# ricosjp/FrontISTR

Hardware: AMD Instinct MI355X
Metric: CG iterations/sec + SpMV achieved HBM GB/s, 10M-DOF 3x3-block mesh (higher is better)
Workload: dtype f64

## Files before the change

### frontistr_amd/csrc/fistr_hip.hip

```cpp
#include <dlfcn.h>
#include <rccl/rccl.h>
#include <stdio.h>
#include <stdlib.h>
#include <string.h>

#include <algorithm>
#include <chrono>
#include <mutex>
#include <thread>

#include "fx_assemble.h"
#include "fx_assemble_tet.h"
#include "fx_assemble_c3.h"
#include "fx_kernels.h"
#include "fx_nonlinear.h"
#include "fx_nonlinear_tet.h"
#include "fx_nonlinear_c3.h"

namespace fxo {
struct Graph {
  int32_t n = 0;
  std::vector<int64_t> ptr;
  std::vector<int32_t> adj;
};
// ... 245 lines not shown
    {"FX_DF_GRID", [](fx_context *c, double v) { c->df_grid = (int)v; }},
    {"FX_DF_POLL", [](fx_context *c, double v) { c->df_poll = (int)v; }},
    {"FX_DF_SLEEP", [](fx_context *c, double v) { c->df_sleep = std::max(0, (int)v); }},
    {"FX_DF_PRESLEEP", [](fx_context *c, double v) { c->df_presleep = std::max(0, (int)v); }},
    {"FX_DF_WPS", [](fx_context *c, double v) { c->df_wps = ((int)v == 2 || (int)v == 4) ? (int)v : 8; }},
    {"FX_MARCH", [](fx_context *c, double v) { c->march_mode = std::max(0, std::min(2, (int)v)); }},
    {"FX_MARCH_CHUNK", [](fx_context *c, double v) { c->march_chunk = std::max(0, (int)v); }},
    {"FX_MARCH_WAVES", [](fx_context *c, double v) { c->march_waves = (int)v; }},
    {"FX_MARCH_GRID", [](fx_context *c, double v) { c->march_grid = std::max(0, (int)v); }},
    {"FX_MARCH_XCD", [](fx_context *c, double v) { c->march_xcd = (int)v != 0; }},
    {"FX_DEBUG_DF_FAIL", [](fx_context *c, double v) { c->dbg_df_fail = (int)v != 0; }},
    {"FX_DEBUG_ONECOLOR", [](fx_context *c, double v) { c->dbg_onecolor = (int)v != 0; }},
    {"FX_SSOR_NATURAL", [](fx_context *c, double v) { c->ssor_natural = (int)v != 0; }},
    {"FX_SPLIT_WPS", [](fx_context *c, double v) { c->split_wps = ((int)v == 2 || (int)v == 4 || (int)v == 8) ? (int)v : 0; }},
};

extern "C" int fx_set_option(fx_context *c, const char *name, double value) {
  if (!c || !name) { g_fx_error = "fx_set_option: null argument"; return FX_ERROR_RUNTIME; }
  for (const FxOption &o : g_fx_options)
    if (strcmp(o.name, name) == 0) {
      const bool spatial = c->spmv_spatial;
      const int bs = c->spmv_bs;
      o.set(c, value);
      if (c->m_symbolic && (spatial != c->spmv_spatial || bs != c->spmv_bs)) {
        HIP_TRY(hipSetDevice(c->device));
        HIP_TRY(hipStreamSynchronize(c->stream));
        return spmv_walk(c);
      }
      return 0;
    }
  g_fx_error = std::string("fx_set_option: unknown option ") + name;
  return FX_ERROR_UNSUPPORTED;
}
// ... 7 lines not shown
    const char *lr = getenv("LOCAL_RANK");
    if (!lr) lr = getenv("OMPI_COMM_WORLD_LOCAL_RANK");
    if (!lr) lr = getenv("MPI_LOCALRANKID");
    if (!lr) lr = getenv("SLURM_LOCALID");
    device = lr ? atoi(lr) % ndev : 0;
  }
  HIP_TRY(hipSetDevice(device));
  fx_context *c = new fx_context();
  c->device = device;
  HIP_TRY(hipDeviceGetAttribute(&c->n_cu, hipDeviceAttributeMultiprocessorCount, device));
  if (context_init(c)) {
    fx_destroy(c);
    return FX_ERROR_RUNTIME;
  }
  for (const FxOption &o : g_fx_options)
    if (const char *e = getenv(o.name)) o.set(c, atof(e));
  {
    int pc[3] = {64, 64, 64};
    auto occ = [&](int k, auto kernel, int threads) {
      int n = 0;
      if (hipOccupancyMaxActiveBlocksPerMultiprocessor(&n, kernel, threads, 0) != hipSuccess) n = 1;
      pc[k] = std::min(pc[k], n);
    };
    occ(0, k_tri_dataflow<2, 1, true>, 128); occ(0, k_tri_dataflow<2, 0, true>, 128); occ(0, k_tri_dataflow<2, 1, false>, 128); occ(0, k_tri_dataflow<2, 0, false>, 128);
    occ(1, k_tri_dataflow<4, 1, true>, 256); occ(1, k_tri_dataflow<4, 0, true>, 256); occ(1, k_tri_dataflow<4, 1, false>, 256); occ(1, k_tri_dataflow<4, 0, false>, 256);
    occ(2, k_tri_dataflow<8, 1, true>, 512); occ(2, k_tri_dataflow<8, 0, true>, 512); occ(2, k_tri_dataflow<8, 1, false>, 512); occ(2, k_tri_dataflow<8, 0, false>, 512);
    (void)hipGetLastError();
    for (int k = 0; k < 3; k++) c->df_grid_max[k] = std::max(1, c->n_cu * std::max(1, std::min(pc[k], 8)));
    int pe[2] = {1, 1};
    if (hipOccupancyMaxActiveBlocksPerMultiprocessor(&pe[0], k_eis_backward_df<4>, 256, 0) != hipSuccess) pe[0] = 1;
    if (hipOccupancyMaxActiveBlocksPerMultiprocessor(&pe[1], k_eis_forward_df<4>, 256, 0) != hipSuccess) pe[1] = 1;
    (void)hipGetLastError();
    for (int k = 0; k < 2; k++) c->eis_df_grid_max[k] = std::max(1, c->n_cu * std::max(1, std::min(pe[k], EIS_DF_MAX_PER_CU)));
    int pm[4] = {1, 1, 1, 1};
    auto occm = [&](int k, auto kernel, int threads) {
      if (hipOccupancyMaxActiveBlocksPerMultiprocessor(&pm[k], kernel, threads, 0) != hipSuccess) pm[k] = 1;
    };
    occm(0, k_tri_march<1>, 64 * 2); occm(1, k_tri_march<2>, 64 * 3); occm(2, k_tri_march<3>, 64 * 4); pm[3] = pm[2];
    (void)hipGetLastError();
    for (int k = 0; k < 4; k++) c->march_grid_max[k] = std::max(8, c->n_cu * std::max(1, std::min(pm[k], 4)));
  }
  *out = c;
  return 0;
}

static void arena_destroy(fx_context *c) {
// ... 1578 lines not shown
    const int s0 = S.color_slice[col], s1 = S.color_slice[col + 1];
    if (s1 <= s0) continue;
    if (s1 - s0 <= c->split_max_slices)
      hipLaunchKernelGGL((k_ssor_color_split<true, 4>), dim3(s1 - s0), dim3(256), 0, c->stream, s0, s1, S.L.pair_ptr, S.L.val2, S.L.col2,
                         (const int32_t *)nullptr, S.alu, rhs, out, (double *)nullptr, (double *)nullptr, gate);
    else if (c->ssor_bs == 64)
      hipLaunchKernelGGL((k_ssor_color<true, true, 64>), dim3((s1 - s0 + spb - 1) / spb), dim3(64), 0, c->stream, s0, s1, S.L.pair_ptr,
                         S.L.val2, S.L.col2, (const int32_t *)nullptr, S.alu, rhs, out, (double *)nullptr, (double *)nullptr, gate, 1);
    else
      hipLaunchKernelGGL((k_ssor_color<true, true, 256>), dim3((s1 - s0 + spb - 1) / spb), dim3(256), 0, c->stream, s0, s1, S.L.pair_ptr,
                         S.L.val2, S.L.col2, (const int32_t *)nullptr, S.alu, rhs, out, (double *)nullptr, (double *)nullptr, gate, 1);
  }
  HIP_TRY(hipGetLastError());
  return 0;
}
static int eis_refresh_t(fx_context *c, const int32_t *gate) {
  SsorDev &S = c->ssor;
  const int32_t ns = c->ord.nslots;
  if (eis_sweep_forward_solve(c, c->W[0], c->W[3], gate)) return FX_ERROR_RUNTIME;
  hipLaunchKernelGGL((k_eis_update<0>), dim3((ns + FX_BLOCK - 1) / FX_BLOCK), dim3(FX_BLOCK), 0, c->stream, ns, c->st, S.alu,
                     (const double *)nullptr, (const double *)nullptr, (const double *)nullptr, (double *)nullptr,
                     (double *)nullptr, c->W[3], c->W[4], c->partials, c->partials + c->max_partials, gate);
  HIP_TRY(hipGetLastError());
  return 0;
}
static int eis_begin(fx_context *c) {
  c->eis_rho_done = false;
  for (int k : {1, 2, 5, 6, 7}) HIP_TRY(hipMemsetAsync(c->W[k], 0, (size_t)c->wlen * 8, c->stream));
  HIP_TRY(hipMemsetAsync(c->W[3], 0, (size_t)c->wlen * 8, c->stream));
  return eis_refresh_t(c, nullptr);
}
static int eis_tail(fx_context *c, int *grid) {
  const SsorDev &S = c->ssor;
  grid[0] = grid[1] = 0;
  if (c->df_mode < 1 || multi_rank(c) || c->nranks > 1 || halo_active(c) || !c->eis_fuse || c->eis_grid > 0 || S.ncolor <= 0)
    return S.ncolor;
  int gk[2];
  for (int k = 0; k < 2; k++) gk[k] = c->df_grid > 0 ? std::min(c->df_grid, c->eis_df_grid_max[k]) : c->eis_df_grid_max[k];
  const int g = std::min(gk[0], gk[1]);
  int c0 = S.ncolor;
  while (c0 > 0) {
    const int nsl = S.color_slice[c0] - S.color_slice[c0 - 1];
    if (nsl > EIS_TAIL_GRIDS * g || nsl > c->split_max_slices) break;
    c0--;
// ... 7 lines not shown
static int eis_cg_iteration(fx_context *c, int it) {
  SsorDev &S = c->ssor;
  const int32_t ns = c->ord.nslots;
  const int64_t n3 = (int64_t)3 * ns;
  double *R = c->W[0], *P = c->W[1], *PH = c->W[2], *T = c->W[3], *DT = c->W[4], *V = c->W[5], *WH = c->W[6], *Q = c->W[7];
  double *X = c->Xs, *B = c->Bs;
  const int RECOMPUTE = 50, vgrid = grid_for(n3, FX_BLOCK, 2048), ugrid = (ns + FX_BLOCK - 1) / FX_BLOCK;
  const double esc = (S.sigma_diag - 1.0) / S.sigma_diag;
  double *part_rho = c->partials + c->max_partials;
  if (!c->eis_rho_done && scalar_stage<OP_CG_RHO>(c, ugrid, 0, RECOMPUTE, part_rho)) return FX_ERROR_RUNTIME;
  c->eis_rho_done = false;
  int tgrid[2];
  const int tc0 = eis_tail(c, tgrid);
  const int ts0 = S.color_slice[tc0], ts1 = S.color_slice[S.ncolor];
  c->eis_tail_color0 = tc0; c->eis_tail_slices = ts1 - ts0; c->eis_tail_grid = tgrid[0];
  if (tc0 < S.ncolor) {
    const int64_t n16 = (int64_t)(ts1 - ts0) * 64 * 3 * 8 / 16;
    hipLaunchKernelGGL(k_eis_tag, dim3(grid_for(n16, 256, 2048)), dim3(256), 0, c->stream, n16, (fx_u4 *)(P + (size_t)3 * 64 * ts0),
                       (fx_u4 *)(V + (size_t)3 * 64 * ts0), gate_status(c));
  }
  if (c->eis_fuse) {
    ClockScope cs(c, 1);
    const int spb = c->ssor_bs / 64;
    if (tc0 < S.ncolor) {
      hipLaunchKernelGGL((k_eis_backward_df<4>), dim3(tgrid[0]), dim3(256), 0, c->stream, ts0, ts1, S.U.pair_ptr, S.U.val2, S.U.col2, S.alu,
                         c->st, DT, PH, P, gate_status(c), c->df_err, c->dbg_df_fail ? 1 : 0);
      c->eis_tail_launches++;
    }
    for (int col = tc0 - 1; col >= 0; col--) {
      const int s0 = S.color_slice[col], s1 = S.color_slice[col + 1];
      if (s1 <= s0) continue;
      if (s1 - s0 <= c->split_max_slices)
        hipLaunchKernelGGL((k_eis_backward_split<4>), dim3(c->eis_grid > 0 ? std::min(s1 - s0, c->eis_grid) : s1 - s0), dim3(256), 0, c->stream, s0, s1, S.U.pair_ptr, S.U.val2, S.U.col2, S.alu,
                           c->st, DT, PH, P, gate_status(c));
      else if (c->ssor_bs == 64)
        hipLaunchKernelGGL((k_eis_backward<64>), dim3((s1 - s0 + spb - 1) / spb), dim3(64), 0, c->stream, s0, s1, S.U.pair_ptr, S.U.val2,
                           S.U.col2, S.alu, c->st, DT, PH, P, gate_status(c));
      else
        hipLaunchKernelGGL((k_eis_backward<256>), dim3((s1 - s0 + spb - 1) / spb), dim3(256), 0, c->stream, s0, s1, S.U.pair_ptr, S.U.val2,
                           S.U.col2, S.alu, c->st, DT, PH, P, gate_status(c));
    }
  } else {
    hipLaunchKernelGGL(k_cg_update_p, dim3(vgrid), dim3(FX_BLOCK), 0, c->stream, n3, c->st, DT, PH);
    if (eis_sweep_backward(c, PH, P, gate_status(c))) return FX_ERROR_RUNTIME;
  }
  const double *HP = nullptr;
  if (halo_active(c)) {
    if (halo_update(c, P)) return FX_ERROR_RUNTIME;
    ClockScope cs(c, 0);
    hipLaunchKernelGGL(k_eis_halo, dim3((S.H.nslices + 3) / 4), dim3(256), 0, c->stream, S.H.nslices, S.H.pair_ptr, S.H.val2, S.H.col2, P,
                       c->W[8], gate_status(c));
    HP = c->W[8];
  }
  {
    ClockScope cs(c, 0);
// ... 15 lines not shown
                           esc, PH, P, V, WH, Q, c->partials, off, gate_status(c), HP);
      off += g;
    }
    if (tc0 < S.ncolor) {
      hipLaunchKernelGGL((k_eis_forward_df<4>), dim3(tgrid[1]), dim3(256), 0, c->stream, ts0, ts1, S.L.pair_ptr, S.L.val2, S.L.col2, S.alu,
                         esc, PH, P, V, WH, Q, c->partials, off, gate_status(c), c->df_err, c->dbg_df_fail ? 1 : 0);
      c->eis_tail_launches++;
      off += ts1 - ts0;
    }
    HIP_TRY(hipGetLastError());
    if (off > c->max_partials) { g_fx_error = "eisenstat: partial-sum buffer too small"; return FX_ERROR_RUNTIME; }
    if (scalar_stage<OP_CG_C1>(c, off, 0, RECOMPUTE)) return FX_ERROR_RUNTIME;
  }
  int np;
  if (it % RECOMPUTE == 0) {
    hipLaunchKernelGGL((k_eis_update<2>), dim3(ugrid), dim3(FX_BLOCK), 0, c->stream, ns, c->st, S.alu, P, Q, WH, X, R, T, DT,
                       c->partials, part_rho, gate_status(c));
    if (spmv(c, 1, 2, X, B, R, gate_status(c), 0)) return FX_ERROR_RUNTIME;
    np = spmv_nparts(c);
    if (scalar_stage<OP_RESID>(c, np, 0, RECOMPUTE)) return FX_ERROR_RUNTIME;
    if (eis_refresh_t(c, gate_status(c))) return FX_ERROR_RUNTIME;
  } else {
    hipLaunchKernelGGL((k_eis_update<1>), dim3(ugrid), dim3(FX_BLOCK), 0, c->stream, ns, c->st, S.alu, P, Q, WH, X, R, T, DT,
                       c->partials, part_rho, gate_status(c));
    if (c->eis_merge) {
      if (scalar_stage<OP_RESID_RHO>(c, ugrid, c->max_partials, RECOMPUTE)) return FX_ERROR_RUNTIME;
      c->eis_rho_done = true;
    } else if (scalar_stage<OP_RESID>(c, ugrid, 0, RECOMPUTE)) return FX_ERROR_RUNTIME;
  }
  HIP_TRY(hipGetLastError());
  return 0;
}

static int krylov_begin(fx_context *c, int method, int maxit, double tol) {
  const int64_t n3 = (int64_t)3 * c->ord.nslots;
  double *X = c->Xs, *B = c->Bs, *R = c->W[0];
  int np;
  if (ensure_solver(c)) return FX_ERROR_RUNTIME;
  if (to_slots(c, c->A.B, c->Bs) || to_slots(c, c->A.X, c->Xs)) return FX_ERROR_RUNTIME;
  c->k_method = method; c->k_maxit = maxit; c->k_it = 1;
  graphs_destroy(c);
  const bool sweepy = (c->precond_kind == 1 || level_sched(c));
  c->k_graph = !c->clock.on && !multi_rank(c) && c->nranks <= 1 && c->halo.n_neighbor <= 0 &&
               (c->graph_mode == 2 || (c->graph_mode == 1 && sweepy && c->ord.nslots <= c->graph_max_rows));
  if (krylov_init_state(c, maxit, tol, true)) return FX_ERROR_RUNTIME;
  HIP_TRY(hipMemsetAsync(c->W[2], 0, (size_t)c->wlen * 8, c->stream));
  if (c->precond_kind == 1 || level_sched(c))
    HIP_TRY(hipMemsetAsync(c->ssor.zs, 0, (size_t)3 * c->ssor.nslots * 8, c->stream));
  if (method == 2) HIP_TRY(hipMemsetAsync(c->W[6], 0, (size_t)c->wlen * 8, c->stream));
  if (spmv(c, 1, 0, X, B, R, nullptr, 0)) return FX_ERROR_RUNTIME;
  if (method == 2) {
    hipLaunchKernelGGL(k_copy, dim3(grid_for(n3, FX_BLOCK, 2048)), dim3(256), 0, c->stream, n3, R, c->W[1]);
  }
  if (dot_into_partials(c, B, B, nullptr, 0, &np)) return FX_ERROR_RUNTIME;
  if (scalar_stage<OP_BNRM2>(c, np, 0, 50)) return FX_ERROR_RUNTIME;
  HIP_TRY(hipGetLastError());
// ... 721 lines not shown
  HIP_TRY(hipEventElapsedTime(&ms, c->ev0, c->ev1));
  *gbs = (double)n2 * 16.0 * nrepeat / (ms * 1e-3) / 1e9;
  return 0;
}


extern "C" int fx_get_stats(fx_context *c, int64_t out[16]) {
  memset(out, 0, 16 * sizeof(int64_t));
  out[0] = c->A.N; out[1] = c->A.NP; out[2] = c->A.NPL; out[3] = c->A.NPU;
  out[4] = c->M.npairs; out[5] = c->M.nblocks; out[6] = c->M.nslices;
  out[7] = c->ssor.ncolor;
  out[8] = c->ssor.L.npairs; out[9] = c->ssor.L.nblocks; out[10] = c->ssor.U.npairs; out[11] = c->ssor.U.nblocks;
  out[12] = c->ssor.L.nslices;
  out[13] = c->M.n_wg_interior; out[14] = c->M.n_wg_boundary;
  out[15] = (c->eis_active ? 1 : 0) | (c->precond_kind == 11 ? 2 : 0) | ((int64_t)(c->df_mode & 3) << 2) | ((int64_t)std::min(c->df_fallbacks, 255) << 8) |
           ((int64_t)c->df_grid_last << 16);
  return 0;
}

extern "C" int fx_eis_tail_stats(fx_context *c, int64_t out[6]) {
  out[0] = c->eis_tail_color0; out[1] = c->eis_tail_slices; out[2] = c->eis_tail_grid; out[3] = c->eis_tail_launches;
  out[4] = c->ssor.ncolor; out[5] = std::min(c->eis_df_grid_max[0], c->eis_df_grid_max[1]);
  return 0;
}

extern "C" int fx_get_ssor_ordering(fx_context *c, int32_t *perm, int32_t *colorindex, int32_t colorindex_cap, int32_t *ncolor) {
  const SsorDev &S = c->ssor;
  if (c->precond_kind != 1 || S.perm.empty()) { g_fx_error = "fx_get_ssor_ordering: no multicolour SSOR resident"; return FX_ERROR_RUNTIME; }
  if ((int32_t)S.colorindex.size() > colorindex_cap) { g_fx_error = "fx_get_ssor_ordering: colorindex too small"; return FX_ERROR_RUNTIME; }
  std::copy(S.perm.begin(), S.perm.end(), perm);
  std::copy(S.colorindex.begin(), S.colorindex.end(), colorindex);
// ... 10 lines not shown
```

### frontistr_amd/csrc/fx_internal.h

```cpp
#pragma once
#include <hip/hip_runtime.h>
#include <stddef.h>
#include <stdint.h>

#include <string>
#include <utility>
#include <vector>

#include "../../include/fistr_hip.h"

extern thread_local std::string g_fx_error;
int fx_fail(const char *what, const char *file, int line);

#define HIP_TRY(expr)                                                        \
  do {                                                                       \
    hipError_t _e = (expr);                                                  \
    if (_e != hipSuccess) {                                                  \
      g_fx_error = std::string(#expr) + ": " + hipGetErrorString(_e);        \
      return fx_fail(g_fx_error.c_str(), __FILE__, __LINE__);                \
    }                                                                        \
  } while (0)

struct DevCSR {
  int32_t N = 0, NP = 0, NPL = 0, NPU = 0;
// ... 255 lines not shown
  bool df_soa = true;
  int df_grid_max[3] = {128, 128, 128};
  int df_grid_last = 0;
  bool dbg_df_fail = false;
  int df_fallbacks = 0;
  int32_t *df_err = nullptr;
  int march_mode = 0, march_chunk = 0, march_waves = 0, march_grid = 0, march_xcd = 1;
  int march_grid_max[4] = {0, 0, 0, 0};
  int march_launches = 0;
  bool pipe_spmv = true, pipe_ssor = true;
  bool eisenstat = true, eis_active = false;
  bool eis_rho_done = false, eis_merge = true;
  int eis_grid = 0;
  bool dbg_onecolor = false;
  bool eis_fuse = true;
  int eis_df_grid_max[2] = {128, 128};
  int eis_tail_color0 = 0, eis_tail_slices = 0, eis_tail_grid = 0;
  int64_t eis_tail_launches = 0;
  int64_t values_epoch = 0;
  bool layout_device = true;
  int32_t mc_batch = 32;
  int32_t mc_device_min = 100000;
  bool val2_pow2 = true;
  DevArena arena;
  int arena_tries = 4;
  double arena_good_gbs = 6450.0;
  std::vector<DevArena> arena_tried;
  std::vector<float> arena_ms;
  bool arena_verified = false;
  size_t arena_min_bytes = (size_t)32 << 30;
// ... 48 lines not shown
```

### frontistr_amd/csrc/fx_kernels.h

```cpp
#pragma once
#include "fx_internal.h"

#define FX_BLOCK 256

__device__ __forceinline__ int xcd_block(int b, int nb) {
  const int q = nb >> 3, r = nb & 7, x = b & 7, k = b >> 3;
  return (x < r ? x * (q + 1) : r * (q + 1) + (x - r) * q) + k;
}

__device__ __forceinline__ double wave_sum(double v) {
#pragma unroll
  for (int off = 32; off > 0; off >>= 1) v += __shfl_down(v, off, 64);
  return v;
}

template <int NV, int BS = FX_BLOCK>
__device__ __forceinline__ void block_sum_store(double (&v)[NV], double *out, int stride, int slot = -1) {
  if (slot < 0) slot = blockIdx.x;
  __shared__ double sm[NV][BS / 64];
  const int lane = threadIdx.x & 63, w = threadIdx.x >> 6;
#pragma unroll
  for (int i = 0; i < NV; i++) {
    double s = wave_sum(v[i]);
    if (lane == 0) sm[i][w] = s;
// ... 191 lines not shown

__device__ __forceinline__ void lumul33_dev(const double *u, double x1, double x2, double x3, double &y1, double &y2, double &y3,
                                            double &d1, double &d2, double &d3) {
  const double p1 = 1.0 / u[0], p2 = 1.0 / u[4], p3 = 1.0 / u[8];
  const double t1 = p1 * x1 + u[1] * x2 + u[2] * x3;
  const double t2 = p2 * x2 + u[5] * x3;
  const double t3 = p3 * x3;
  y1 = t1;
  y2 = u[3] * t1 + t2;
  y3 = u[6] * t1 + u[7] * t2 + t3;
  d1 = p1;
  d2 = u[3] * u[1] + p2;
  d3 = u[6] * u[2] + u[7] * u[5] + p3;
}

__global__ void k_alu_setup(int32_t nslots, int32_t nrows, const int32_t *__restrict__ slot_row,
                            const double *__restrict__ D, double sigma_diag, double *__restrict__ alu) {
  const int slot = blockIdx.x * blockDim.x + threadIdx.x;
  if (slot >= nslots) return;
  const int row = slot_row ? slot_row[slot] : slot;
  double a[9] = {1, 0, 0, 0, 1, 0, 0, 0, 1};
  if (row >= 0 && row < nrows) {
#pragma unroll
    for (int e = 0; e < 9; e++) a[e] = D[(size_t)9 * row + e];
    a[0] *= sigma_diag; a[4] *= sigma_diag; a[8] *= sigma_diag;
    lu33_dev(a);
  }
  const size_t base = (size_t)(slot >> 6) * 576 + (slot & 63);
#pragma unroll
  for (int e = 0; e < 9; e++) alu[base + (size_t)e * 64] = a[e];
// ... 362 lines not shown
      for (int k = 0; k < 3; k++) { sv[k] = part[0][k][lane]; sp[k] = part[0][3 + k][lane]; }
#pragma unroll
      for (int j = 1; j < WPS; j++)
#pragma unroll
        for (int k = 0; k < 3; k++) { sv[k] += part[j][k][lane]; sp[k] += part[j][3 + k][lane]; }
      dsum += eis_forward_finish(slice, lane, sv, sp, alu, esc, ph, p, v, w, q, hp);
    }
    if (slice + (int)gridDim.x < slice1) __syncthreads();
  }
  if (wv == 0) {
    dsum = wave_sum(dsum);
    if (lane == 0) partials[part0 + blockIdx.x] = dsum;
  }
}

__device__ __forceinline__ void eis_backward_finish(int slice, int lane, double s0, double s1, double s2, const double *__restrict__ alu,
                                                    const KrylovState *__restrict__ st, const double *__restrict__ dt,
                                                    double *__restrict__ ph, double *__restrict__ p) {
  const size_t o = (size_t)3 * (slice * 64 + lane);
  double u[9];
  const size_t base = (size_t)slice * 576 + lane;
#pragma unroll
  for (int e = 0; e < 9; e++) u[e] = alu[base + (size_t)e * 64];
  double h0 = dt[o], h1 = dt[o + 1], h2 = dt[o + 2];
  if (st->iter != 1) {
    const double beta = st->beta;
    h0 = h0 + beta * ph[o]; h1 = h1 + beta * ph[o + 1]; h2 = h2 + beta * ph[o + 2];
  }
  ph[o] = h0; ph[o + 1] = h1; ph[o + 2] = h2;
  double x1 = h0 - s0, x2 = h1 - s1, x3 = h2 - s2;
  lusolve33_dev(u, x1, x2, x3);
  p[o] = x1; p[o + 1] = x2; p[o + 2] = x3;
}

template <int BS>
__global__ __launch_bounds__(BS) void k_eis_backward(int32_t slice0, int32_t slice1, const int32_t *__restrict__ pair_ptr,
                                                     const double *__restrict__ val2, const int *__restrict__ col2,
                                                     const double *__restrict__ alu, const KrylovState *__restrict__ st,
                                                     const double *__restrict__ dt, double *__restrict__ ph, double *__restrict__ p,
                                                     const int32_t *__restrict__ gate) {
  if (gate && *gate != 0) return;
  const int vb = xcd_block(blockIdx.x, gridDim.x);
  const int slice = slice0 + vb * (BS / 64) + (threadIdx.x >> 6);
  const int lane = threadIdx.x & 63;
  if (slice >= slice1) return;
  double s0 = 0.0, s1 = 0.0, s2 = 0.0;
  bell_row_sweep<true>(pair_ptr[slice], pair_ptr[slice + 1], val2, col2, lane, p, s0, s1, s2);
  eis_backward_finish(slice, lane, s0, s1, s2, alu, st, dt, ph, p);
}

template <bool PUB>
__device__ __forceinline__ void eis_backward_finish_own(size_t o, const double (&fu)[9], const double (&fd)[3], const double (&fp)[3],
                                                        double s0, double s1, double s2, const KrylovState *__restrict__ st,
                                                        double *__restrict__ ph, double *p) {
  double g0 = fd[0], g1 = fd[1], g2 = fd[2];
  if (st->iter != 1) {
    const double beta = st->beta;
    g0 = g0 + beta * fp[0]; g1 = g1 + beta * fp[1]; g2 = g2 + beta * fp[2];
  }
  ph[o] = g0; ph[o + 1] = g1; ph[o + 2] = g2;
  double x1 = g0 - s0, x2 = g1 - s1, x3 = g2 - s2;
  lusolve33_dev(fu, x1, x2, x3);
  if (PUB) {
    df_store(p + o, x1); df_store(p + o + 1, x2); df_store(p + o + 2, x3);
  } else {
    p[o] = x1; p[o + 1] = x2; p[o + 2] = x3;
  }
}

template <int WPS>
__global__ __launch_bounds__(64 * WPS) void k_eis_backward_split(int32_t slice0, int32_t slice1, const int32_t *__restrict__ pair_ptr,
                                                                 const double *__restrict__ val2, const int *__restrict__ col2,
                                                                 const double *__restrict__ alu, const KrylovState *__restrict__ st,
                                                                 const double *__restrict__ dt, double *__restrict__ ph,
                                                                 double *__restrict__ p, const int32_t *__restrict__ gate) {
  __shared__ double part[WPS][3][64];
  const int lane = threadIdx.x & 63, w = threadIdx.x >> 6;
  if (gate && *gate != 0) return;
  for (int slice = slice0 + blockIdx.x; slice < slice1; slice += gridDim.x) {
    const int h0 = pair_ptr[slice], h1 = pair_ptr[slice + 1];
    const int np = (h1 - h0) >> 1;
    double s0 = 0.0, s1 = 0.0, s2 = 0.0;
    double fu[9], fd[3], fp[3];
    if (w == 0) {
      const size_t o = (size_t)3 * (slice * 64 + lane), base = (size_t)slice * 576 + lane;
// ... 16 lines not shown
    if (((h1 - h0) & 1) && w == (np % WPS)) {
      const double *vt = val2 + (size_t)(h0 + 2 * np) * 576 + lane;
      const int cc = ld_stream(col2 + (size_t)(h0 + 2 * np) * 64 + lane);
      double a[9];
#pragma unroll
      for (int e = 0; e < 9; e++) a[e] = ld_stream(vt + e * 64);
      const double x[3] = {p[(size_t)3 * cc], p[(size_t)3 * cc + 1], p[(size_t)3 * cc + 2]};
      bell_single_fma(a, x, s0, s1, s2);
    }
    part[w][0][lane] = s0; part[w][1][lane] = s1; part[w][2][lane] = s2;
    __syncthreads();
    if (w == 0) {
      s0 = part[0][0][lane]; s1 = part[0][1][lane]; s2 = part[0][2][lane];
#pragma unroll
      for (int k = 1; k < WPS; k++) { s0 += part[k][0][lane]; s1 += part[k][1][lane]; s2 += part[k][2][lane]; }
      eis_backward_finish_own<false>((size_t)3 * (slice * 64 + lane), fu, fd, fp, s0, s1, s2, st, ph, p);
    }
    if (slice + (int)gridDim.x < slice1) __syncthreads();
  }
}

__global__ __launch_bounds__(256) void k_eis_halo(int32_t nslices, const int32_t *__restrict__ pair_ptr, const double *__restrict__ val2,
                                                  const int *__restrict__ col2, const double *__restrict__ p, double *__restrict__ hp,
                                                  const int32_t *__restrict__ gate) {
  if (gate && *gate != 0) return;
  const int slice = blockIdx.x * 4 + (threadIdx.x >> 6), lane = threadIdx.x & 63;
  if (slice >= nslices) return;
  double s0 = 0.0, s1 = 0.0, s2 = 0.0;
  bell_row_sweep<false>(pair_ptr[slice], pair_ptr[slice + 1], val2, col2, lane, p, s0, s1, s2);
  const size_t o = (size_t)3 * (slice * 64 + lane);
  hp[o] = s0; hp[o + 1] = s1; hp[o + 2] = s2;
}

template <int MODE>
__global__ __launch_bounds__(FX_BLOCK) void k_eis_update(int32_t nslots, const KrylovState *__restrict__ st,
                                                         const double *__restrict__ alu, const double *__restrict__ p,
                                                         const double *__restrict__ q, const double *__restrict__ w,
                                                         double *__restrict__ x, double *__restrict__ r, double *__restrict__ t,
                                                         double *__restrict__ dt, double *__restrict__ part_rr,
                                                         double *__restrict__ part_rho, const int32_t *__restrict__ gate) {
  if (gate && *gate != 0) return;
  const int slot = blockIdx.x * FX_BLOCK + threadIdx.x;
  double d[2] = {0.0, 0.0};
  if (slot < nslots) {
    const size_t o = (size_t)3 * slot;
    if (MODE == 2) {
      const double alpha = st->alpha;
      x[o] += alpha * p[o]; x[o + 1] += alpha * p[o + 1]; x[o + 2] += alpha * p[o + 2];
    } else {
      double t0 = t[o], t1 = t[o + 1], t2 = t[o + 2];
      if (MODE == 1) {
        const double alpha = st->alpha;
        x[o] += alpha * p[o]; x[o + 1] += alpha * p[o + 1]; x[o + 2] += alpha * p[o + 2];
        const double r0 = r[o] - alpha * q[o], r1 = r[o + 1] - alpha * q[o + 1], r2 = r[o + 2] - alpha * q[o + 2];
        r[o] = r0; r[o + 1] = r1; r[o + 2] = r2;
        d[0] = r0 * r0 + r1 * r1 + r2 * r2;
        t0 -= alpha * w[o]; t1 -= alpha * w[o + 1]; t2 -= alpha * w[o + 2];
        t[o] = t0; t[o + 1] = t1; t[o + 2] = t2;
      }
      double u[9];
      const size_t base = (size_t)(slot >> 6) * 576 + (slot & 63);
#pragma unroll
      for (int e = 0; e < 9; e++) u[e] = alu[base + (size_t)e * 64];
      double y0, y1, y2, dd0, dd1, dd2;
      lumul33_dev(u, t0, t1, t2, y0, y1, y2, dd0, dd1, dd2);
      dt[o] = y0; dt[o + 1] = y1; dt[o + 2] = y2;
      d[1] = t0 * y0 + t1 * y1 + t2 * y2;
    }
  }
  if (MODE == 2) return;
  __shared__ double sm[2][FX_BLOCK / 64];
  const int lane = threadIdx.x & 63, wv = threadIdx.x >> 6;
  const double s0 = wave_sum(d[0]), s1 = wave_sum(d[1]);
  if (lane == 0) { sm[0][wv] = s0; sm[1][wv] = s1; }
  __syncthreads();
  if (threadIdx.x == 0) {
    double a = 0.0, b = 0.0;
#pragma unroll
    for (int k = 0; k < FX_BLOCK / 64; k++) { a += sm[0][k]; b += sm[1][k]; }
    if (MODE == 1) part_rr[blockIdx.x] = a;
    part_rho[blockIdx.x] = b;
  }
// ... 45 lines not shown
  }
}

__global__ __launch_bounds__(256) void k_eis_tag(int64_t n16, fx_u4 *__restrict__ a, fx_u4 *__restrict__ b, const int32_t *__restrict__ gate) {
  if (gate && *gate != 0) return;
  const fx_u4 tag = {0xFFFFFFFFu, 0xFFFFFFFFu, 0xFFFFFFFFu, 0xFFFFFFFFu};
  for (int64_t i = (int64_t)blockIdx.x * 256 + threadIdx.x; i < n16; i += (int64_t)gridDim.x * 256) {
    asm volatile("global_store_dwordx4 %0, %1, off sc1" ::"v"(a + i), "v"(tag) : "memory");
    asm volatile("global_store_dwordx4 %0, %1, off sc1\n\ts_nop 1" ::"v"(b + i), "v"(tag) : "memory");
  }
}

#define EIS_DF_BLOCKS_BWD 3
#define EIS_DF_BLOCKS_FWD 3

template <int WPS>
__global__ __launch_bounds__(64 * WPS, EIS_DF_BLOCKS_BWD) void k_eis_backward_df(int32_t s0, int32_t s1, const int32_t *__restrict__ pair_ptr,
                                                              const double *__restrict__ val2, const int *__restrict__ col2,
                                                              const double *__restrict__ alu, const KrylovState *__restrict__ st,
                                                              const double *__restrict__ dt, double *__restrict__ ph, double *p,
                                                              const int32_t *__restrict__ gate, int32_t *__restrict__ err, int fail) {
  if (gate && *gate != 0) return;
  if (fail) {
    if (blockIdx.x == 0 && threadIdx.x == 0) __hip_atomic_store(err, 1, __ATOMIC_RELAXED, __HIP_MEMORY_SCOPE_AGENT);
    return;
  }
  __shared__ double part[2][WPS][3][64];
  const int lane = threadIdx.x & 63, w = threadIdx.x >> 6, tail0 = s0 * 64;
  bool dead = false;
  int buf = 0;
  for (int slice = s1 - 1 - (int)blockIdx.x; slice >= s0; slice -= gridDim.x, buf ^= 1) {
// ... 28 lines not shown
    if (((h1 - h0) & 1) && w == (np % WPS)) {
      const double *vt = val2 + (size_t)(h0 + 2 * np) * 576 + lane;
      const int cols[1] = {ld_stream(col2 + (size_t)(h0 + 2 * np) * 64 + lane)};
      double a[9], x[3];
#pragma unroll
      for (int e = 0; e < 9; e++) a[e] = ld_stream(vt + e * 64);
      eis_df_gather<1>(p, cols, self, tail0, x, err, dead);
      bell_single_fma(a, x, s0v, s1v, s2v);
    }
    part[buf][w][0][lane] = s0v; part[buf][w][1][lane] = s1v; part[buf][w][2][lane] = s2v;
    __syncthreads();
    if (w == 0) {
      s0v = part[buf][0][0][lane]; s1v = part[buf][0][1][lane]; s2v = part[buf][0][2][lane];
#pragma unroll
      for (int k = 1; k < WPS; k++) { s0v += part[buf][k][0][lane]; s1v += part[buf][k][1][lane]; s2v += part[buf][k][2][lane]; }
      eis_backward_finish_own<true>((size_t)3 * self, fu, fd, fp, s0v, s1v, s2v, st, ph, p);
    }
  }
}

template <int WPS>
__global__ __launch_bounds__(64 * WPS, EIS_DF_BLOCKS_FWD) void k_eis_forward_df(int32_t s0, int32_t s1, const int32_t *__restrict__ pair_ptr,
                                                             const double *__restrict__ val2, const int *__restrict__ col2,
                                                             const double *__restrict__ alu, double esc,
                                                             const double *__restrict__ ph, const double *__restrict__ p, double *v,
                                                             double *__restrict__ w, double *__restrict__ q,
                                                             double *__restrict__ partials, int32_t part0,
                                                             const int32_t *__restrict__ gate, int32_t *__restrict__ err, int fail) {
  if (gate && *gate != 0) return;
  if (fail) {
    if (blockIdx.x == 0 && threadIdx.x == 0) __hip_atomic_store(err, 1, __ATOMIC_RELAXED, __HIP_MEMORY_SCOPE_AGENT);
// ... 1120 lines not shown
```

### frontistr_amd/hecmw.py

```python
import ctypes as C
import os

import numpy as np

_HERE = os.path.dirname(os.path.abspath(__file__))
LIBPATH = os.path.join(_HERE, "libfistr_hip.so")
_lib = None

HECMW_SOLVER_ERROR_INCONS_PC = 1001
HECMW_SOLVER_ERROR_ZERO_DIAG = 2001
HECMW_SOLVER_ERROR_ZERO_RHS = 2002
HECMW_SOLVER_ERROR_NOCONV_MAXIT = 3001
HECMW_SOLVER_ERROR_DIVERGE_MAT = 3002
HECMW_SOLVER_ERROR_DIVERGE_PC = 3003

FX_UP_PROFILE, FX_UP_VALUES, FX_UP_RHS, FX_UP_X, FX_UP_ALL = 1, 2, 4, 8, 15


class HecmwSolverError(RuntimeError):
    def __init__(self, code, msg):
        super().__init__("HEC-MW-SOLVER %d: %s" % (code, msg))
        self.code = code


# ... 262 lines not shown

    def stream_ceiling_gbs(self, nrepeat=5):
        out = C.c_double(0)
        _chk(lib().fx_stream_ceiling(self.h, nrepeat, C.byref(out)))
        return out.value

    def stats(self):
        out = (C.c_int64 * 16)()
        _chk(lib().fx_get_stats(self.h, out))
        keys = ("N", "NP", "NPL", "NPU", "M_pairs", "M_blocks", "M_slices", "ncolor", "L_pairs", "L_blocks",
                "U_pairs", "U_blocks", "ssor_slices", "wg_interior", "wg_boundary", "eisenstat")
        st = {k: int(out[i]) for i, k in enumerate(keys)}
        v = st["eisenstat"]
        st["ssor_natural"] = (v >> 1) & 1
        st["df_mode"] = (v >> 2) & 3
        st["df_fallbacks"] = (v >> 8) & 0xFF
        st["df_grid"] = v >> 16
        st["eisenstat"] = v & 1
        return st

    def eis_tail_stats(self):
        out = (C.c_int64 * 6)()
        _chk(lib().fx_eis_tail_stats(self.h, out))
        keys = ("color0", "slices", "grid", "launches", "ncolor", "grid_max")
        return {k: int(out[i]) for i, k in enumerate(keys)}

    def krylov_begin(self, hecMAT):
        _chk(lib().fx_krylov_begin(self.h, _ptr(hecMAT.Iarray), _ptr(hecMAT.Rarray)))

    def krylov_steps(self, nsteps):
# ... 326 lines not shown
```

Measured before the change: 570.7.

## Add lean Eisenstat path: recompute D^-1 t in backward sweep, fuse sentinel tagging into update

Adds an on-by-default lean mode for the Eisenstat-preconditioned CG. The update kernel no longer writes the dt = D^-1 t vector. The backward sweep kernels recompute it from t and the per-slot 3x3 LU block when they finish. The dataflow sentinel tags for the tail colors are written by the update kernel itself rather than by a separate tagging kernel. The aim is to cut one full-vector write and read per iteration plus a kernel launch, at the cost of extra FLOPs and alu reads in the backward sweep. It also needs extra tag initialization and cleanup at begin and end.

```diff
diff --git a/frontistr_amd/csrc/fistr_hip.hip b/frontistr_amd/csrc/fistr_hip.hip
--- a/frontistr_amd/csrc/fistr_hip.hip
+++ b/frontistr_amd/csrc/fistr_hip.hip
@@ -283,9 +283,17 @@
     {"FX_SSOR_NATURAL", [](fx_context *c, double v) { c->ssor_natural = (int)v != 0; }},
     {"FX_SPLIT_WPS", [](fx_context *c, double v) { c->split_wps = ((int)v == 2 || (int)v == 4 || (int)v == 8) ? (int)v : 0; }},
 };
+static const FxOption g_fx_eis_switches[] = {
+    {"FX_EIS_LEAN", [](fx_context *c, double v) { c->eis_lean = (int)v != 0; }},
+};
 
 extern "C" int fx_set_option(fx_context *c, const char *name, double value) {
   if (!c || !name) { g_fx_error = "fx_set_option: null argument"; return FX_ERROR_RUNTIME; }
+  for (const FxOption &o : g_fx_eis_switches)
+    if (strcmp(o.name, name) == 0) {
+      o.set(c, value);
+      return 0;
+    }
   for (const FxOption &o : g_fx_options)
     if (strcmp(o.name, name) == 0) {
       const bool spatial = c->spmv_spatial;
@@ -323,6 +331,8 @@
     return FX_ERROR_RUNTIME;
   }
   for (const FxOption &o : g_fx_options)
+    if (const char *e = getenv(o.name)) o.set(c, atof(e));
+  for (const FxOption &o : g_fx_eis_switches)
     if (const char *e = getenv(o.name)) o.set(c, atof(e));
   {
     int pc[3] = {64, 64, 64};
@@ -336,9 +346,14 @@
     occ(2, k_tri_dataflow<8, 1, true>, 512); occ(2, k_tri_dataflow<8, 0, true>, 512); occ(2, k_tri_dataflow<8, 1, false>, 512); occ(2, k_tri_dataflow<8, 0, false>, 512);
     (void)hipGetLastError();
     for (int k = 0; k < 3; k++) c->df_grid_max[k] = std::max(1, c->n_cu * std::max(1, std::min(pc[k], 8)));
-    int pe[2] = {1, 1};
-    if (hipOccupancyMaxActiveBlocksPerMultiprocessor(&pe[0], k_eis_backward_df<4>, 256, 0) != hipSuccess) pe[0] = 1;
-    if (hipOccupancyMaxActiveBlocksPerMultiprocessor(&pe[1], k_eis_forward_df<4>, 256, 0) != hipSuccess) pe[1] = 1;
+    int pe[2] = {64, 64};
+    auto occe = [&](int k, auto kernel) {
+      int n = 0;
+      if (hipOccupancyMaxActiveBlocksPerMultiprocessor(&n, kernel, 256, 0) != hipSuccess) n = 1;
+      pe[k] = std::min(pe[k], n);
+    };
+    occe(0, k_eis_backward_df<4, false>); occe(0, k_eis_backward_df<4, true>);
+    occe(1, k_eis_forward_df<4>);
     (void)hipGetLastError();
     for (int k = 0; k < 2; k++) c->eis_df_grid_max[k] = std::max(1, c->n_cu * std::max(1, std::min(pe[k], EIS_DF_MAX_PER_CU)));
     int pm[4] = {1, 1, 1, 1};
@@ -1947,20 +1962,36 @@
   HIP_TRY(hipGetLastError());
   return 0;
 }
+static bool eis_lean(const fx_context *c) { return c->eis_lean && c->eis_fuse; }
 static int eis_refresh_t(fx_context *c, const int32_t *gate) {
   SsorDev &S = c->ssor;
   const int32_t ns = c->ord.nslots;
   if (eis_sweep_forward_solve(c, c->W[0], c->W[3], gate)) return FX_ERROR_RUNTIME;
-  hipLaunchKernelGGL((k_eis_update<0>), dim3((ns + FX_BLOCK - 1) / FX_BLOCK), dim3(FX_BLOCK), 0, c->stream, ns, c->st, S.alu,
-                     (const double *)nullptr, (const double *)nullptr, (const double *)nullptr, (double *)nullptr,
-                     (double *)nullptr, c->W[3], c->W[4], c->partials, c->partials + c->max_partials, gate);
+  const auto upd = eis_lean(c) ? k_eis_update<0, true> : k_eis_update<0, false>;
+  hipLaunchKernelGGL(upd, dim3((ns + FX_BLOCK - 1) / FX_BLOCK), dim3(FX_BLOCK), 0, c->stream, ns, c->st, S.alu,
+                     (double *)nullptr, (const double *)nullptr, (const double *)nullptr, (double *)nullptr,
+                     (double *)nullptr, c->W[3], c->W[4], c->partials, c->partials + c->max_partials, gate, ns, (double *)nullptr);
   HIP_TRY(hipGetLastError());
   return 0;
 }
+static int eis_tail(fx_context *c, int *grid);
 static int eis_begin(fx_context *c) {
   c->eis_rho_done = false;
+  c->eis_lean_on = eis_lean(c);
   for (int k : {1, 2, 5, 6, 7}) HIP_TRY(hipMemsetAsync(c->W[k], 0, (size_t)c->wlen * 8, c->stream));
   HIP_TRY(hipMemsetAsync(c->W[3], 0, (size_t)c->wlen * 8, c->stream));
+  if (c->eis_lean_on) {
+    const SsorDev &S = c->ssor;
+    int tgrid[2];
+    const int tc0 = eis_tail(c, tgrid);
+    if (tc0 < S.ncolor) {
+      const int ts0 = S.color_slice[tc0], ts1 = S.color_slice[S.ncolor];
+      const int64_t n16 = (int64_t)(ts1 - ts0) * 64 * 3 * 8 / 16;
+      hipLaunchKernelGGL(k_eis_tag, dim3(grid_for(n16, 256, 2048)), dim3(256), 0, c->stream, n16, (fx_u4 *)(c->W[1] + (size_t)3 * 64 * ts0),
+                         (fx_u4 *)(c->W[5] + (size_t)3 * 64 * ts0), (const int32_t *)nullptr);
+      c->eis_tags_left = true;
+    }
+  }
   return eis_refresh_t(c, nullptr);
 }
 static int eis_tail(fx_context *c, int *grid) {
@@ -1998,7 +2029,10 @@
   const int tc0 = eis_tail(c, tgrid);
   const int ts0 = S.color_slice[tc0], ts1 = S.color_slice[S.ncolor];
   c->eis_tail_color0 = tc0; c->eis_tail_slices = ts1 - ts0; c->eis_tail_grid = tgrid[0];
-  if (tc0 < S.ncolor) {
+  const bool lean = c->eis_lean_on;
+  const int32_t tag0 = (lean && tc0 < S.ncolor) ? ts0 * 64 : ns;
+  const double *TD = lean ? T : DT;
+  if (tc0 < S.ncolor && !lean) {
     const int64_t n16 = (int64_t)(ts1 - ts0) * 64 * 3 * 8 / 16;
     hipLaunchKernelGGL(k_eis_tag, dim3(grid_for(n16, 256, 2048)), dim3(256), 0, c->stream, n16, (fx_u4 *)(P + (size_t)3 * 64 * ts0),
                        (fx_u4 *)(V + (size_t)3 * 64 * ts0), gate_status(c));
@@ -2007,22 +2041,22 @@
     ClockScope cs(c, 1);
     const int spb = c->ssor_bs / 64;
     if (tc0 < S.ncolor) {
-      hipLaunchKernelGGL((k_eis_backward_df<4>), dim3(tgrid[0]), dim3(256), 0, c->stream, ts0, ts1, S.U.pair_ptr, S.U.val2, S.U.col2, S.alu,
-                         c->st, DT, PH, P, gate_status(c), c->df_err, c->dbg_df_fail ? 1 : 0);
+      hipLaunchKernelGGL((lean ? k_eis_backward_df<4, true> : k_eis_backward_df<4, false>), dim3(tgrid[0]), dim3(256), 0, c->stream, ts0, ts1, S.U.pair_ptr, S.U.val2, S.U.col2, S.alu,
+                         c->st, TD, PH, P, gate_status(c), c->df_err, c->dbg_df_fail ? 1 : 0);
       c->eis_tail_launches++;
     }
     for (int col = tc0 - 1; col >= 0; col--) {
       const int s0 = S.color_slice[col], s1 = S.color_slice[col + 1];
       if (s1 <= s0) continue;
       if (s1 - s0 <= c->split_max_slices)
-        hipLaunchKernelGGL((k_eis_backward_split<4>), dim3(c->eis_grid > 0 ? std::min(s1 - s0, c->eis_grid) : s1 - s0), dim3(256), 0, c->stream, s0, s1, S.U.pair_ptr, S.U.val2, S.U.col2, S.alu,
-                           c->st, DT, PH, P, gate_status(c));
+        hipLaunchKernelGGL((lean ? k_eis_backward_split<4, true> : k_eis_backward_split<4, false>), dim3(c->eis_grid > 0 ? std::min(s1 - s0, c->eis_grid) : s1 - s0), dim3(256), 0, c->stream, s0, s1, S.U.pair_ptr, S.U.val2, S.U.col2, S.alu,
+                           c->st, TD, PH, P, gate_status(c));
       else if (c->ssor_bs == 64)
-        hipLaunchKernelGGL((k_eis_backward<64>), dim3((s1 - s0 + spb - 1) / spb), dim3(64), 0, c->stream, s0, s1, S.U.pair_ptr, S.U.val2,
-                           S.U.col2, S.alu, c->st, DT, PH, P, gate_status(c));
+        hipLaunchKernelGGL((lean ? k_eis_backward<64, true> : k_eis_backward<64, false>), dim3((s1 - s0 + spb - 1) / spb), dim3(64), 0, c->stream, s0, s1, S.U.pair_ptr, S.U.val2,
+                           S.U.col2, S.alu, c->st, TD, PH, P, gate_status(c));
       else
-        hipLaunchKernelGGL((k_eis_backward<256>), dim3((s1 - s0 + spb - 1) / spb), dim3(256), 0, c->stream, s0, s1, S.U.pair_ptr, S.U.val2,
-                           S.U.col2, S.alu, c->st, DT, PH, P, gate_status(c));
+        hipLaunchKernelGGL((lean ? k_eis_backward<256, true> : k_eis_backward<256, false>), dim3((s1 - s0 + spb - 1) / spb), dim3(256), 0, c->stream, s0, s1, S.U.pair_ptr, S.U.val2,
+                           S.U.col2, S.alu, c->st, TD, PH, P, gate_status(c));
     }
   } else {
     hipLaunchKernelGGL(k_cg_update_p, dim3(vgrid), dim3(FX_BLOCK), 0, c->stream, n3, c->st, DT, PH);
@@ -2068,15 +2102,15 @@
   }
   int np;
   if (it % RECOMPUTE == 0) {
-    hipLaunchKernelGGL((k_eis_update<2>), dim3(ugrid), dim3(FX_BLOCK), 0, c->stream, ns, c->st, S.alu, P, Q, WH, X, R, T, DT,
-                       c->partials, part_rho, gate_status(c));
+    hipLaunchKernelGGL((lean ? k_eis_update<2, true> : k_eis_update<2, false>), dim3(ugrid), dim3(FX_BLOCK), 0, c->stream, ns, c->st, S.alu, P, Q, WH, X, R, T, DT,
+                       c->partials, part_rho, gate_status(c), tag0, V);
     if (spmv(c, 1, 2, X, B, R, gate_status(c), 0)) return FX_ERROR_RUNTIME;
     np = spmv_nparts(c);
     if (scalar_stage<OP_RESID>(c, np, 0, RECOMPUTE)) return FX_ERROR_RUNTIME;
     if (eis_refresh_t(c, gate_status(c))) return FX_ERROR_RUNTIME;
   } else {
-    hipLaunchKernelGGL((k_eis_update<1>), dim3(ugrid), dim3(FX_BLOCK), 0, c->stream, ns, c->st, S.alu, P, Q, WH, X, R, T, DT,
-                       c->partials, part_rho, gate_status(c));
+    hipLaunchKernelGGL((lean ? k_eis_update<1, true> : k_eis_update<1, false>), dim3(ugrid), dim3(FX_BLOCK), 0, c->stream, ns, c->st, S.alu, P, Q, WH, X, R, T, DT,
+                       c->partials, part_rho, gate_status(c), tag0, V);
     if (c->eis_merge) {
       if (scalar_stage<OP_RESID_RHO>(c, ugrid, c->max_partials, RECOMPUTE)) return FX_ERROR_RUNTIME;
       c->eis_rho_done = true;
@@ -2094,6 +2128,10 @@
   if (to_slots(c, c->A.B, c->Bs) || to_slots(c, c->A.X, c->Xs)) return FX_ERROR_RUNTIME;
   c->k_method = method; c->k_maxit = maxit; c->k_it = 1;
   graphs_destroy(c);
+  if (c->eis_tags_left) {
+    for (int k : {1, 5}) HIP_TRY(hipMemsetAsync(c->W[k], 0, (size_t)c->wlen * 8, c->stream));
+    c->eis_tags_left = false;
+  }
   const bool sweepy = (c->precond_kind == 1 || level_sched(c));
   c->k_graph = !c->clock.on && !multi_rank(c) && c->nranks <= 1 && c->halo.n_neighbor <= 0 &&
                (c->graph_mode == 2 || (c->graph_mode == 1 && sweepy && c->ord.nslots <= c->graph_max_rows));
@@ -2845,7 +2883,8 @@
   out[12] = c->ssor.L.nslices;
   out[13] = c->M.n_wg_interior; out[14] = c->M.n_wg_boundary;
   out[15] = (c->eis_active ? 1 : 0) | (c->precond_kind == 11 ? 2 : 0) | ((int64_t)(c->df_mode & 3) << 2) | ((int64_t)std::min(c->df_fallbacks, 255) << 8) |
-           ((int64_t)c->df_grid_last << 16);
+           ((int64_t)c->df_grid_last << 16) |
+           ((c->eis_active && c->eis_lean_on) ? 16 : 0);
   return 0;
 }
 
diff --git a/frontistr_amd/csrc/fx_internal.h b/frontistr_amd/csrc/fx_internal.h
--- a/frontistr_amd/csrc/fx_internal.h
+++ b/frontistr_amd/csrc/fx_internal.h
@@ -293,6 +293,7 @@
   int eis_grid = 0;
   bool dbg_onecolor = false;
   bool eis_fuse = true;
+  bool eis_lean = true, eis_lean_on = false, eis_tags_left = false;
   int eis_df_grid_max[2] = {128, 128};
   int eis_tail_color0 = 0, eis_tail_slices = 0, eis_tail_grid = 0;
   int64_t eis_tail_launches = 0;
diff --git a/frontistr_amd/csrc/fx_kernels.h b/frontistr_amd/csrc/fx_kernels.h
--- a/frontistr_amd/csrc/fx_kernels.h
+++ b/frontistr_amd/csrc/fx_kernels.h
@@ -229,6 +229,16 @@
   d3 = u[6] * u[2] + u[7] * u[5] + p3;
 }
 
+__device__ __forceinline__ void lumul33_pinned_dev(const double *u, double x1, double x2, double x3, double &y1, double &y2, double &y3,
+                                                   double &xy) {
+  const double p1 = 1.0 / u[0], p2 = 1.0 / u[4], p3 = 1.0 / u[8];
+  y1 = __builtin_fma(x3, u[2], __builtin_fma(x2, u[1], x1 * p1));
+  const double t2 = __builtin_fma(x3, u[5], x2 * p2);
+  y2 = __builtin_fma(u[3], y1, t2);
+  y3 = __builtin_fma(x3, p3, __builtin_fma(u[7], t2, u[6] * y1));
+  xy = __builtin_fma(x3, y3, __builtin_fma(x1, y1, x2 * y2));
+}
+
 __global__ void k_alu_setup(int32_t nslots, int32_t nrows, const int32_t *__restrict__ slot_row,
                             const double *__restrict__ D, double sigma_diag, double *__restrict__ alu) {
   const int slot = blockIdx.x * blockDim.x + threadIdx.x;
@@ -621,6 +631,7 @@
   }
 }
 
+template <bool LEAN>
 __device__ __forceinline__ void eis_backward_finish(int slice, int lane, double s0, double s1, double s2, const double *__restrict__ alu,
                                                     const KrylovState *__restrict__ st, const double *__restrict__ dt,
                                                     double *__restrict__ ph, double *__restrict__ p) {
@@ -630,6 +641,11 @@
 #pragma unroll
   for (int e = 0; e < 9; e++) u[e] = alu[base + (size_t)e * 64];
   double h0 = dt[o], h1 = dt[o + 1], h2 = dt[o + 2];
+  if (LEAN) {
+    double y0, y1, y2, ty;
+    lumul33_pinned_dev(u, h0, h1, h2, y0, y1, y2, ty);
+    h0 = y0; h1 = y1; h2 = y2;
+  }
   if (st->iter != 1) {
     const double beta = st->beta;
     h0 = h0 + beta * ph[o]; h1 = h1 + beta * ph[o + 1]; h2 = h2 + beta * ph[o + 2];
@@ -640,7 +656,7 @@
   p[o] = x1; p[o + 1] = x2; p[o + 2] = x3;
 }
 
-template <int BS>
+template <int BS, bool LEAN>
 __global__ __launch_bounds__(BS) void k_eis_backward(int32_t slice0, int32_t slice1, const int32_t *__restrict__ pair_ptr,
                                                      const double *__restrict__ val2, const int *__restrict__ col2,
                                                      const double *__restrict__ alu, const KrylovState *__restrict__ st,
@@ -653,14 +669,19 @@
   if (slice >= slice1) return;
   double s0 = 0.0, s1 = 0.0, s2 = 0.0;
   bell_row_sweep<true>(pair_ptr[slice], pair_ptr[slice + 1], val2, col2, lane, p, s0, s1, s2);
-  eis_backward_finish(slice, lane, s0, s1, s2, alu, st, dt, ph, p);
-}
-
-template <bool PUB>
+  eis_backward_finish<LEAN>(slice, lane, s0, s1, s2, alu, st, dt, ph, p);
+}
+
+template <bool PUB, bool LEAN>
 __device__ __forceinline__ void eis_backward_finish_own(size_t o, const double (&fu)[9], const double (&fd)[3], const double (&fp)[3],
                                                         double s0, double s1, double s2, const KrylovState *__restrict__ st,
                                                         double *__restrict__ ph, double *p) {
   double g0 = fd[0], g1 = fd[1], g2 = fd[2];
+  if (LEAN) {
+    double y0, y1, y2, ty;
+    lumul33_pinned_dev(fu, g0, g1, g2, y0, y1, y2, ty);
+    g0 = y0; g1 = y1; g2 = y2;
+  }
   if (st->iter != 1) {
     const double beta = st->beta;
     g0 = g0 + beta * fp[0]; g1 = g1 + beta * fp[1]; g2 = g2 + beta * fp[2];
@@ -675,7 +696,7 @@
   }
 }
 
-template <int WPS>
+template <int WPS, bool LEAN>
 __global__ __launch_bounds__(64 * WPS) void k_eis_backward_split(int32_t slice0, int32_t slice1, const int32_t *__restrict__ pair_ptr,
                                                                  const double *__restrict__ val2, const int *__restrict__ col2,
                                                                  const double *__restrict__ alu, const KrylovState *__restrict__ st,
@@ -722,7 +743,7 @@
       s0 = part[0][0][lane]; s1 = part[0][1][lane]; s2 = part[0][2][lane];
 #pragma unroll
       for (int k = 1; k < WPS; k++) { s0 += part[k][0][lane]; s1 += part[k][1][lane]; s2 += part[k][2][lane]; }
-      eis_backward_finish_own<false>((size_t)3 * (slice * 64 + lane), fu, fd, fp, s0, s1, s2, st, ph, p);
+      eis_backward_finish_own<false, LEAN>((size_t)3 * (slice * 64 + lane), fu, fd, fp, s0, s1, s2, st, ph, p);
     }
     if (slice + (int)gridDim.x < slice1) __syncthreads();
   }
@@ -740,13 +761,14 @@
   hp[o] = s0; hp[o + 1] = s1; hp[o + 2] = s2;
 }
 
-template <int MODE>
+template <int MODE, bool LEAN>
 __global__ __launch_bounds__(FX_BLOCK) void k_eis_update(int32_t nslots, const KrylovState *__restrict__ st,
-                                                         const double *__restrict__ alu, const double *__restrict__ p,
+                                                         const double *__restrict__ alu, double *p,
                                                          const double *__restrict__ q, const double *__restrict__ w,
                                                          double *__restrict__ x, double *__restrict__ r, double *__restrict__ t,
                                                          double *__restrict__ dt, double *__restrict__ part_rr,
-                                                         double *__restrict__ part_rho, const int32_t *__restrict__ gate) {
+                                                         double *__restrict__ part_rho, const int32_t *__restrict__ gate, int32_t tag0,
+                                                         double *__restrict__ v) {
   if (gate && *gate != 0) return;
   const int slot = blockIdx.x * FX_BLOCK + threadIdx.x;
   double d[2] = {0.0, 0.0};
@@ -759,7 +781,8 @@
       double t0 = t[o], t1 = t[o + 1], t2 = t[o + 2];
       if (MODE == 1) {
         const double alpha = st->alpha;
-        x[o] += alpha * p[o]; x[o + 1] += alpha * p[o + 1]; x[o + 2] += alpha * p[o + 2];
+        const double p0 = p[o], p1 = p[o + 1], p2 = p[o + 2];
+        x[o] += alpha * p0; x[o + 1] += alpha * p1; x[o + 2] += alpha * p2;
         const double r0 = r[o] - alpha * q[o], r1 = r[o + 1] - alpha * q[o + 1], r2 = r[o + 2] - alpha * q[o + 2];
         r[o] = r0; r[o + 1] = r1; r[o + 2] = r2;
         d[0] = r0 * r0 + r1 * r1 + r2 * r2;
@@ -770,10 +793,23 @@
       const size_t base = (size_t)(slot >> 6) * 576 + (slot & 63);
 #pragma unroll
       for (int e = 0; e < 9; e++) u[e] = alu[base + (size_t)e * 64];
-      double y0, y1, y2, dd0, dd1, dd2;
-      lumul33_dev(u, t0, t1, t2, y0, y1, y2, dd0, dd1, dd2);
-      dt[o] = y0; dt[o + 1] = y1; dt[o + 2] = y2;
-      d[1] = t0 * y0 + t1 * y1 + t2 * y2;
+      if (LEAN) {
+        double y0, y1, y2;
+        lumul33_pinned_dev(u, t0, t1, t2, y0, y1, y2, d[1]);
+      } else {
+        double y0, y1, y2, dd0, dd1, dd2;
+        lumul33_dev(u, t0, t1, t2, y0, y1, y2, dd0, dd1, dd2);
+        dt[o] = y0; dt[o + 1] = y1; dt[o + 2] = y2;
+        d[1] = t0 * y0 + t1 * y1 + t2 * y2;
+      }
+    }
+    if (LEAN && MODE != 0 && slot >= tag0) {
+      const double tag = __longlong_as_double(FX_DF_SENTINEL);
+#pragma unroll
+      for (int k = 0; k < 3; k++) {
+        __hip_atomic_store(p + o + k, tag, __ATOMIC_RELAXED, __HIP_MEMORY_SCOPE_AGENT);
+        __hip_atomic_store(v + o + k, tag, __ATOMIC_RELAXED, __HIP_MEMORY_SCOPE_AGENT);
+      }
     }
   }
   if (MODE == 2) return;
@@ -849,7 +885,7 @@
 #define EIS_DF_BLOCKS_BWD 3
 #define EIS_DF_BLOCKS_FWD 3
 
-template <int WPS>
+template <int WPS, bool LEAN>
 __global__ __launch_bounds__(64 * WPS, EIS_DF_BLOCKS_BWD) void k_eis_backward_df(int32_t s0, int32_t s1, const int32_t *__restrict__ pair_ptr,
                                                               const double *__restrict__ val2, const int *__restrict__ col2,
                                                               const double *__restrict__ alu, const KrylovState *__restrict__ st,
@@ -908,7 +944,7 @@
       s0v = part[buf][0][0][lane]; s1v = part[buf][0][1][lane]; s2v = part[buf][0][2][lane];
 #pragma unroll
       for (int k = 1; k < WPS; k++) { s0v += part[buf][k][0][lane]; s1v += part[buf][k][1][lane]; s2v += part[buf][k][2][lane]; }
-      eis_backward_finish_own<true>((size_t)3 * self, fu, fd, fp, s0v, s1v, s2v, st, ph, p);
+      eis_backward_finish_own<true, LEAN>((size_t)3 * self, fu, fd, fp, s0v, s1v, s2v, st, ph, p);
     }
   }
 }
diff --git a/frontistr_amd/hecmw.py b/frontistr_amd/hecmw.py
--- a/frontistr_amd/hecmw.py
+++ b/frontistr_amd/hecmw.py
@@ -300,6 +300,7 @@
         v = st["eisenstat"]
         st["ssor_natural"] = (v >> 1) & 1
         st["df_mode"] = (v >> 2) & 3
+        st["eis_lean"] = (v >> 4) & 1
         st["df_fallbacks"] = (v >> 8) & 0xFF
         st["df_grid"] = v >> 16
         st["eisenstat"] = v & 1
```

After: 573.3, median of 6. About the same (+0.4%).
